# YuanchenBei/ColdRec

Hardware: AMD Instinct MI355X
Metric: ranked items/sec (full-catalogue eval) (higher is better)
Workload: dtype f32; 1 GPU; configs[3] full-catalogue eval: 1000000-row user table x 10000000 items, d=128, k=20, f32 tables, user block 131072 per step, rated CSR (mean ~50) + 20% cold-item bitmap ('warm' setting), item table row-sharded over 1 GPU(s); items=10000000, dim=128, k=20, parallelism=single GPU

## Files before the change

### coldrec_amd/csrc/score_topk.hip

```cpp
#include <math.h>
#include <stdarg.h>
#include <stdlib.h>

#include <algorithm>
#include <atomic>
#include <vector>

#include "score_topk_common.h"

using namespace crh_score;

namespace {

__device__ __forceinline__ bool pack_row_masked(const uint32_t* bitmap, int64_t gid) {
    return bitmap != nullptr && ((bitmap[gid >> 5] >> (gid & 31)) & 1u);
}

template <int D>
__global__ __launch_bounds__(256) void pack_items_kernel(const float* __restrict__ v, int64_t n_items,
                                                         float* __restrict__ packed, const uint32_t* __restrict__ bitmap,
                                                         int64_t item_base) {
    constexpr int NCH = D / 8;
    __shared__ float tile[32][D + 4];
    const int64_t t = blockIdx.x;
// ... 949 lines not shown
        unsigned long long t0 = ~0ull, t1 = 0;
        for (int64_t wv = 0; wv < n_waves; ++wv) { t0 = std::min(t0, h[2 * wv]); t1 = std::max(t1, h[2 * wv + 1]); }
        std::vector<double> st_(n_waves), en_(n_waves);
        for (int64_t wv = 0; wv < n_waves; ++wv) { st_[wv] = (double)(h[2 * wv] - t0); en_[wv] = (double)(h[2 * wv + 1] - t0); }
        std::sort(st_.begin(), st_.end());
        std::sort(en_.begin(), en_.end());
        const double tot = (double)(t1 - t0);
        fprintf(stderr, "[crh timing] waves=%lld span=%.0f ticks; start quantiles 0/25/50/75/100%%: %.3f %.3f %.3f %.3f %.3f; "
                        "end quantiles 0/10/25/50/75/90/100%%: %.3f %.3f %.3f %.3f %.3f %.3f %.3f (fraction of span)\n",
                (long long)n_waves, tot, st_[0] / tot, st_[n_waves / 4] / tot, st_[n_waves / 2] / tot,
                st_[3 * n_waves / 4] / tot, st_[n_waves - 1] / tot, en_[0] / tot, en_[n_waves / 10] / tot,
                en_[n_waves / 4] / tot, en_[n_waves / 2] / tot, en_[3 * n_waves / 4] / tot, en_[9 * n_waves / 10] / tot,
                en_[n_waves - 1] / tot);
        std::vector<double> in_(n_waves), lp_(n_waves), so_(n_waves);
        double ev_ticks = 0, ev = 0, lp_sum = 0;
        for (int64_t wv = 0; wv < n_waves; ++wv) {
            in_[wv] = (double)(h[2 * n_waves + 2 * wv] - h[2 * wv]);
            lp_[wv] = (double)(h[2 * n_waves + 2 * wv + 1] - h[2 * n_waves + 2 * wv]);
            so_[wv] = (double)(h[2 * wv + 1] - h[2 * n_waves + 2 * wv + 1]);
            ev_ticks += (double)h[4 * n_waves + 2 * wv];
            ev += (double)h[4 * n_waves + 2 * wv + 1];
            lp_sum += lp_[wv];
        }
        std::sort(in_.begin(), in_.end());
        std::sort(lp_.begin(), lp_.end());
        std::sort(so_.begin(), so_.end());
        fprintf(stderr, "[crh timing] median ticks: list setup %.0f, tile loop %.0f, list store %.0f; %.0f slow-path events per wave, "
                        "%.0f ticks each = %.3f of the loop\n",
                in_[n_waves / 2], lp_[n_waves / 2], so_[n_waves / 2], ev / (double)n_waves, ev > 0 ? ev_ticks / ev : 0.0,
                lp_sum > 0 ? ev_ticks / lp_sum : 0.0);
    return CRH_OK;
}
int dma_timing_begin(ScoreArgs& a, hipStream_t st) {
    CRH_HIP(hipMalloc(&a.wave_clock, (size_t)16 * 4 * 68 * 8));
    CRH_HIP(hipMemsetAsync(a.wave_clock, 0, (size_t)16 * 4 * 68 * 8, st));
    return CRH_OK;
}
int dma_timing_report(ScoreArgs& a, int esz, int d, hipStream_t st) {
    CRH_HIP(hipStreamSynchronize(st));
    std::vector<unsigned long long> h((size_t)16 * 4 * 68);
    CRH_HIP(hipMemcpy(h.data(), a.wave_clock, h.size() * 8, hipMemcpyDeviceToHost));
    CRH_HIP(hipFree(a.wave_clock));
    {
        unsigned long long tk = 0, ne = 0;
        for (int q = 0; q < 64; ++q) { tk += h[(size_t)16 * 4 * 64 + 2 * q]; ne += h[(size_t)16 * 4 * 64 + 2 * q + 1]; }
        fprintf(stderr, "[crh dma timing] events: %.0f per wave, %.0f cycles each (tiles with at least one candidate; 64 waves)\n",
                (double)ne / 64.0, ne ? (double)tk / (double)ne : 0.0);
    }
    unsigned long long trip_tk = 0, trip_n = 0, loop_cycles = 0;
    for (int wv = 0; wv < 4; ++wv) {
        unsigned long long tot = 0, wsum = 0;
        std::vector<unsigned long long> b(64, 0);
        for (int blk = 0; blk < 16; ++blk)
            for (int q = 0; q < 64; ++q) b[q] += h[((size_t)blk * 4 + wv) * 64 + q];
        const unsigned long long bw = (esz == 4 ? 512 : 128) >> (d * esz == 256 ? 1 : 0);
        for (int q = 0; q < 64; ++q) { tot += b[q]; wsum += b[q] * (q * bw + bw / 2); }
        fprintf(stderr, "[crh dma timing] wave %d: %llu tiles, mean %.0f cycles; histogram (%llu-cycle buckets from 0):", wv, tot,
                tot ? (double)wsum / (double)tot : 0.0, bw);
        for (int q = 0; q < 64; ++q) fprintf(stderr, " %llu", b[q]);
        fprintf(stderr, "\n");
        loop_cycles += 2 * wsum;
    }
    for (int q = 0; q < 64; ++q) { trip_tk += h[(size_t)16 * 4 * 66 + 2 * q]; trip_n += h[(size_t)16 * 4 * 66 + 2 * q + 1]; }
    fprintf(stderr, "[crh dma timing] memory trips inside events (filter hit -> list bounds + search): %.0f per wave, %.0f cycles each, "
                    "%.0f cycles per wave = %.4f of the timed tile loop (64 waves)\n",
            (double)trip_n / 64.0, trip_n ? (double)trip_tk / (double)trip_n : 0.0, (double)trip_tk / 64.0,
            loop_cycles ? (double)trip_tk / (double)loop_cycles : 0.0);
    a.wave_clock = nullptr;
    return CRH_OK;
}
#endif

int score_topk_impl(int esz, const void* user_emb, const int32_t* users, int64_t n_users, const void* item_emb,
                    int64_t n_items, int d, const int64_t* rated_rowptr, const int32_t* rated_col,
                    const uint32_t* cand_bitmap, int k, int64_t item_base, float* out_score, int32_t* out_idx,
                    void* workspace, size_t workspace_bytes, void* stream, int n_splits, void* ev_kernel_start,
                    void* ev_kernel_stop, const char* who, const float* seed_score, const int32_t* seed_idx) {
    CRH_CHECK_ARG(user_emb && item_emb && out_score && out_idx, "%s: NULL table/output pointer", who);
    CRH_CHECK_ARG(n_users > 0 && n_items > 0, "%s: empty block (n_users=%lld, n_items=%lld)", who,
                  (long long)n_users, (long long)n_items);
    CRH_CHECK_ARG(k >= 1 && k <= CRH_MAX_K, "%s: k=%d outside 1..%d", who, k, CRH_MAX_K);
    CRH_CHECK_ARG(esz == 4 ? crh_score_topk_supports_dim(d) : crh_score_topk_f16_supports_dim(d),
                  "%s: d=%d unsupported (pad the tables to %s16/32/64/128/256)", who, d, esz == 4 ? "8/" : "");
    CRH_CHECK_ARG(((uintptr_t)user_emb & 15) == 0 && ((uintptr_t)item_emb & 15) == 0,
                  "%s: tables must be 16-byte aligned", who);
    CRH_CHECK_ARG((rated_rowptr == nullptr) == (rated_col == nullptr) || rated_rowptr != nullptr,
                  "%s: rated_col given without rated_rowptr", who);
    CRH_CHECK_ARG(item_base >= 0 && item_base + n_items < (int64_t)CRH_PAD_IDX, "%s: item ids exceed int32", who);
    CRH_CHECK_ARG(n_splits >= 0 && n_splits <= 64, "%s: n_splits=%d outside 0..64", who, n_splits);

    const RoutePlan rp = plan_route(esz, n_users, n_items, d, k, workspace != nullptr, workspace_bytes, cand_bitmap != nullptr,
                                    n_splits, seed_score != nullptr);
    ScoreArgs a = {};
    a.user_emb = user_emb;
    a.users = users;
    a.n_users = n_users;
    a.item_emb = item_emb;
    a.n_items = n_items;
    a.rated_rowptr = rated_rowptr;
    a.rated_col = rated_col;
// ... 280 lines not shown
        a.out_idx = reinterpret_cast<int32_t*>(a.out_score + (size_t)a.n_splits * n_users * KP);
    }
    static const int sync_win_raw = CRH_TUNE_ENV("CRH_SCORE_SYNC_WINDOW") ? atoi(CRH_TUNE_ENV("CRH_SCORE_SYNC_WINDOW")) : 128;
    static const int sync_win = sync_win_raw <= 0 ? 0 : std::max(2, sync_win_raw & ~1);
    if (sync_win > 0 && a.n_splits == 1 && n_wg <= 256 && n_wg > 8) {
        const int64_t n_win = (T + 1 + sync_win - 1) / sync_win + 1;
        if ((size_t)(n_win + 1) * 8 * sizeof(unsigned) <= sync_bytes(n_items)) {
            a.sync_window = sync_win;
            a.sync_stride = n_win + 1;
            a.xcd_sync = reinterpret_cast<unsigned*>(ws + L.sync);
            CRH_HIP(hipMemsetAsync(a.xcd_sync, 0, (size_t)a.sync_stride * 8 * sizeof(unsigned), st));
        }
    }
    if (compact) {
        a.idmap = stream_map;
        a.n_live = s.stats + SCREEN_STAT_LIVE;
        if (plan.rated_tiles) {
            int32_t* inv = reinterpret_cast<int32_t*>(ws + L.inv);
            uint32_t* rt = reinterpret_cast<uint32_t*>(ws + L.rtiles);
            rc = launch_screen_invmap(stream_map, a.n_live, item_base + P, n_main, inv, st);
            if (rc != CRH_OK) return rc;
            rc = launch_screen_rated_tiles(rated_rowptr, rated_col, n_users, cand_bitmap, item_base + P, item_base + n_items, inv, rt, st);
            if (rc != CRH_OK) return rc;
            a.rated_tiles = rt;
        }
    } else if (cand_bitmap) {
        a.tile_bits = tbits;
    }
#ifdef CRH_PROFILE
    static const int timing = CRH_PROFILE_ENV("CRH_SCORE_TIMING");
    if (timing) {
        rc = dma_timing_begin(a, st);
        if (rc != CRH_OK) return rc;
    }
#endif
    rc = launch_score_dma(2, D, 3, a, st);
    if (rc != CRH_OK) return rc;
#ifdef CRH_PROFILE
    if (timing) {
        rc = dma_timing_report(a, 2, D, st);
        if (rc != CRH_OK) return rc;
    }
#endif
    if (a.n_splits > 1) {
        rc = crh_merge_topk(a.out_score, a.out_idx, a.n_splits, n_users, KP, KP, cand_s, cand_i, stream);
        if (rc != CRH_OK) return rc;
    }

    rc = launch_screen_certify(s, st);
    if (rc != CRH_OK) return rc;
    if (ev_kernel_stop) CRH_HIP(hipEventRecord(reinterpret_cast<hipEvent_t>(ev_kernel_stop), st));
    return CRH_OK;
}
}

namespace {
size_t full_workspace_bytes(int64_t n_users, int64_t n_items, int d, int k, int esz, bool dim_ok) {
    if (n_users <= 0 || k <= 0) return 0;
    const size_t lists = lists_bytes(n_users, k);
    const size_t fused = dim_ok && n_items > 0 ? fused_layout(n_users, n_items, d, k, esz).need : lists;
    size_t need = std::max(fused, dense_block_bytes(n_users, n_items) + (fused - lists));
    const int64_t P = dim_ok ? seed_route(esz, n_users, n_items, d) : 0;
    if (P > 0) need = std::max(need, dense_block_bytes(n_users, P) + packed_bytes(P, d, esz)) + seed_bytes(n_users, k);
    return need;
}
}
// ... 224 lines not shown
```

### coldrec_amd/csrc/score_topk_dma.hip

```cpp
#include <type_traits>
#include <utility>

#include "score_topk_common.h"

namespace crh_score {
namespace {

constexpr int DMA_NW = 4;
constexpr int DMA_UPW = 128;
constexpr int TBITS_B = 2 * 64 * 4;
constexpr int FLAGS_B = 64;
constexpr int IDS_SLOTS = 8;
constexpr int IDS_B = (IDS_SLOTS + 1) * 32 * 4;
constexpr int RT_B = 2 * 256;

constexpr int DMA_FW = 6;
__host__ __device__ constexpr size_t dma_wave_lds_bytes(int K) {
    return (size_t)DMA_UPW * K * 8 + (size_t)DMA_UPW * 4 + (size_t)DMA_UPW * DMA_FW * 4;
}
__device__ __forceinline__ unsigned rated_hash192(int gi) { return ((((unsigned)gi * 2654435761u) >> 16) * (32u * DMA_FW)) >> 16; }

template <int K>
__device__ __forceinline__ float f4_comp(const f32x4& v) {
    if constexpr (K == 0) return v.x;
// ... 99 lines not shown
            lsu[p] = sc;
            liu[p] = gi;
            cnt[ul] = n2;
        }
        if (n2 >= K) {
            const float prev = __builtin_bit_cast(float, __builtin_amdgcn_readlane(__builtin_bit_cast(int, es), K >= 2 ? K - 2 : 0));
            const float kth = (p == K - 1) ? sc : prev;
            const float t = dma_new_tau<MG>(kth, es, sc, a.screen_k < 2 ? 2 : a.screen_k, margin);
            if (mine) tau_reg = t;
        }
    }
}

#ifdef CRH_DMA_EVENT_REBALLOT
constexpr bool DMA_EVENT_REBALLOT = true;
#else
constexpr bool DMA_EVENT_REBALLOT = false;
#endif
#ifdef CRH_DMA_SCREEN_TWO_TRIP
constexpr bool DMA_SCREEN_ONE_TRIP = false;
#else
constexpr bool DMA_SCREEN_ONE_TRIP = true;
#endif
#ifdef CRH_DMA_SCREEN_MFMA32
constexpr bool DMA_SCREEN_M16 = false;
#else
constexpr bool DMA_SCREEN_M16 = true;
#endif
#ifdef CRH_DMA_M16_BODY_OLD
constexpr bool DMA_M16_HOOKED = false;
#else
constexpr bool DMA_M16_HOOKED = true;
#endif
#ifdef CRH_DMA_EVENT_RUNTIME_K
constexpr int DMA_EVENT_KC = 0;
#else
constexpr int DMA_EVENT_KC = SCREEN_KP;
#endif
#ifdef CRH_DMA_EVENT_SLOT_TEST
constexpr bool DMA_EVENT_SLOT_TEST = true;
#else
constexpr bool DMA_EVENT_SLOT_TEST = false;
#endif
#ifdef CRH_DMA_EVENT_TAIL64
constexpr bool DMA_EVENT_TAIL64 = true;
#else
constexpr bool DMA_EVENT_TAIL64 = false;
#endif
#ifdef CRH_DMA_EVENT_MASK8_SPLIT
[[maybe_unused]] constexpr bool DMA_EVENT_MASK8_SPLIT = true;
#else
[[maybe_unused]] constexpr bool DMA_EVENT_MASK8_SPLIT = false;
#endif
#ifdef CRH_DMA_EVENT_NO_FULL
constexpr bool DMA_EVENT_FULL = false;
#else
constexpr bool DMA_EVENT_FULL = DMA_EVENT_KC != 0 && DMA_SCREEN_ONE_TRIP;
#endif
#ifdef CRH_DMA_EVENT_NO_STRAIGHT
constexpr bool DMA_EVENT_STRAIGHT = false;
#else
constexpr bool DMA_EVENT_STRAIGHT = true;
#endif
template <int K, bool RT>
__device__ __forceinline__ void dma_candidate_full(float sc, int gi, bool bm_masked, int ul, int64_t slot, float* ls, int* li,
                                                   const ScoreArgs& a, int lane, const unsigned* rfilter, bool mine, float& tau_reg,
// ... 160 lines not shown
    while (lanes) {
        const int L = __builtin_ctzll(lanes);
        lanes &= lanes - 1;
        unsigned cmL = __builtin_amdgcn_readlane(cm, L);
        const unsigned bmL = __builtin_amdgcn_readlane(bm, L);
        if constexpr (DMA_EVENT_SLOT_TEST) {
            if (slot0 + (L & 15) >= a.n_users) continue;
        }
        while (cmL) {
            const int r = __builtin_ctz(cmL);
            cmL &= cmL - 1;
            candidate(L, r, bmL);
        }
    }
}


template <typename T, int D, int R, bool FL, bool CM = false, bool M16 = false>
__global__ __launch_bounds__(256, 1) void score_topk_dma_kernel(ScoreArgs a) {
    constexpr int NW = DMA_NW, UW = 4, UPW = DMA_UPW;
    static_assert(!M16 || (std::is_same<T, _Float16>::value && D == 128 && !FL), "the 16x16x32 form is the fp16 d=128 screen's");
    constexpr int UB = M16 ? 16 : 32, NU = UPW / UB, NR = M16 ? 8 : 16;
    using AccT = std::conditional_t<M16, f32x8, f32x16>;
    constexpr int PF = FL ? 2 : 3;
    static_assert(R == 4 && (!FL || sizeof(T) == 4) && !(CM && FL), "ring shape");
    constexpr int SIDE_B = CM ? IDS_B + RT_B : TBITS_B;
    constexpr int ROWB = D * (int)sizeof(T);
    constexpr int NCH = ROWB / 32;
    constexpr int TILE_B = NCH * 1024;
    constexpr int CPW = NCH / NW;
    constexpr int GR = 2, NG = NCH / GR;
    constexpr int BG = NG / 2 - 1;
    constexpr int TG = M16 ? 2 : 1;
    static_assert(NCH % NW == 0 && NG % 4 == 0 && BG + 2 < NG, "row width not supported by the DMA kernel");
    extern __shared__ __attribute__((aligned(16))) char smem[];

    const int lane = threadIdx.x & 63;
    const int wave = __builtin_amdgcn_readfirstlane((int)(threadIdx.x >> 6));
    const int S = a.n_splits;
    const int split = (int)(blockIdx.x % S);
    const int64_t ug_raw = (int64_t)(blockIdx.x / S) * NW + wave;
    const bool live = ug_raw < a.n_ugroups;
    const int64_t ug = live ? ug_raw : a.n_ugroups - 1;
    constexpr int KC = M16 ? DMA_EVENT_KC : 0;
    const int K = KC ? KC : a.k;
    const int i = lane & (M16 ? 15 : 31), h = lane >> (M16 ? 4 : 5);
    constexpr bool MG = std::is_same<T, _Float16>::value && D == 128;

    char* ring = smem;
    unsigned* tbits = reinterpret_cast<unsigned*>(smem + R * TILE_B);
    [[maybe_unused]] unsigned* rtiles = tbits + IDS_B / 4;
    unsigned* flags = tbits + SIDE_B / 4;
    if constexpr (FL) {
        if (threadIdx.x < 16) flags[threadIdx.x] = threadIdx.x < PF - 1 ? (unsigned)NW : 0u;
    }
    int64_t n_rows = a.n_items;
    if constexpr (CM) n_rows = (int64_t)__builtin_amdgcn_readfirstlane((int)*a.n_live);
    const int64_t NT = (n_rows + 31) >> 5;
    const int64_t t0 = NT * split / S, t1 = NT * (split + 1) / S;
    const int64_t split_end = (t1 << 5) < n_rows ? (t1 << 5) : n_rows;
    const int64_t slot0w = ug * UPW;
    auto cut_ids = [&](int& lo, int& hi) __attribute__((always_inline)) {
        if constexpr (CM) {
            const int id_end = (int)(a.item_base + a.n_items);
            if (S == 1) {
                lo = (int)a.item_base;
// ... 195 lines not shown
    auto flag_bump = [&](int word) __attribute__((always_inline)) {
#if defined(__HIP_DEVICE_COMPILE__)
        asm volatile("ds_add_u32 %0, %1" ::"v"(flags_lds + 4u * (unsigned)word), "v"(bump_val) : "memory");
#endif
    };
    auto flag_land = [&](unsigned& f) __attribute__((always_inline)) {
#if defined(__HIP_DEVICE_COMPILE__)
        asm volatile("s_waitcnt lgkmcnt(0)" : "+v"(f));
#endif
    };
    auto lds_wait_fl = [&](f32x4(&x)[GR], unsigned& f0, unsigned& f1) __attribute__((always_inline)) {
#if defined(__HIP_DEVICE_COMPILE__)
        asm volatile("s_waitcnt lgkmcnt(%4)" : "+v"(x[0]), "+v"(x[1]), "+v"(f0), "+v"(f1) : "i"(GR));
#endif
    };
    auto flag_spin = [&](unsigned have, int word, unsigned want) __attribute__((always_inline)) {
        unsigned v = __builtin_amdgcn_readfirstlane(have);
        if (__builtin_expect(v >= want, 1) || (CRH_ABLATE(a.ablate) & 4)) return;
        unsigned spins = 0;
        do {
            __builtin_amdgcn_s_sleep(1);
            unsigned t;
#if defined(__HIP_DEVICE_COMPILE__)
            asm volatile("ds_read_b32 %0, %1\n\ts_waitcnt lgkmcnt(0)" : "=v"(t) : "v"(flags_lds + 4u * (unsigned)word) : "memory");
#endif
            v = __builtin_amdgcn_readfirstlane(t);
            if (++spins > (1u << 24)) __builtin_trap();
        } while (v < want);
    };

#ifdef CRH_PROFILE
    unsigned long long ev_ticks = 0, ev_count = 0;
    DmaTripProf tp = {0ull, 0ull};
#endif
    auto event16 = [&](const AccT& v, float& tau_u, int u, int64_t ts, int rows_left, int gi0, unsigned tb, int idv, bool rt) __attribute__((always_inline)) {
        if constexpr (M16) {
            if constexpr (FULL_FORM) {
                if (lists_full) {
                    tile_slow_path_dma16<CM, KC, true>(v, tau_u, ls, li, cnt, K, UB * u, slot0w + UB * u, a, ts << 5, split_end, rows_left, gi0,
                                                       lane, tb, rfilter, idv, margin, rt CRH_TRIP_ARG);
                    return;
                }
            }
            tile_slow_path_dma16<CM, KC>(v, tau_u, ls, li, cnt, K, UB * u, slot0w + UB * u, a, ts << 5, split_end, rows_left, gi0, lane, tb,
                                         rfilter, idv, margin, rt CRH_TRIP_ARG);
        }
    };
    auto body = [&](auto Pc, int j, int s_cur, int s_nxt, int s_fill) __attribute__((always_inline)) {
        constexpr int P = decltype(Pc)::value, Q = 1 - P;
        const uint32_t src = ring_lds + s_cur * TILE_B, srcn = ring_lds + s_nxt * TILE_B;
        float m[NU];
        auto group = [&](auto Gc) __attribute__((always_inline)) {
            constexpr int g = decltype(Gc)::value;
            if constexpr (g + 2 < NG) lds_group(c[(g + 2) & 3], src, std::integral_constant<int, g + 2>{});
            else lds_group(c[(g + 2) & 3], srcn, std::integral_constant<int, g + 2 - NG>{});
            if constexpr (!FL && g == BG) {
                dma_wait_but_newest_tile();
                if (!(CRH_ABLATE(a.ablate) & 4)) __builtin_amdgcn_s_barrier();
            }
            __builtin_amdgcn_sched_barrier(0);
            if constexpr (FL) {
                lds_wait_fl(c[g & 3], rflag, dflag);
            } else {
                lds_wait(c[g & 3], std::integral_constant<int, 2 * GR>{});
            }
            if constexpr (!FL && g == BG) {
// ... 117 lines not shown
                    if constexpr (CM) idv = (int)tbits[((j - 1) & (IDS_SLOTS - 1)) * 32 + (lane & 31)];
                    bool rt = false;
                    if constexpr (CM) rt = (__builtin_amdgcn_readfirstlane(rtiles[(int)((ts >> 9) & 1) * 64 + (int)((ts >> 3) & 63)]) >> (4 * (int)(ts & 7) + wave)) & 1u;
                    const int64_t rl64 = split_end - (ts << 5);
                    const int rows_left = rl64 < 32 ? (int)rl64 : 32;
                    const int gi0 = (int)(a.item_base + (ts << 5));
#pragma unroll
                    for (int u = 0; u < NU; ++u)
                        if ((M16 && !DMA_EVENT_REBALLOT) ? hitb[u] != 0ull : __ballot(m[u] > tau[u]) != 0ull) {
                            if constexpr (M16)
                                event16(acc[Q][u], tau[u], u, ts, rows_left, gi0, tb, idv, rt);
                            else
                                tile_slow_path_dma<sizeof(T) == 4 && DMA_ONE_TRIP_F32, CM, MG>(acc[Q][u], tau[u], ls, li, cnt, K, 32 * u, slot0w + 32 * u, a,
                                                                                                ts << 5, split_end, lane, tb, rfilter, idv, margin, rt CRH_TRIP_ARG);
                        }
                    __builtin_amdgcn_s_waitcnt(0xc07f);
#ifdef CRH_PROFILE
                    if (a.wave_clock != nullptr) {
                        ev_ticks += __builtin_amdgcn_s_memtime() - ev_t0;
                        ev_count += 1;
                    }
#endif
                }
            }
        };
        [&]<int... Gs>(std::integer_sequence<int, Gs...>) __attribute__((always_inline)) {
            (group(std::integral_constant<int, Gs>{}), ...);
        }(std::make_integer_sequence<int, NG>{});
    };

    uint32_t ring_a = ring_lds;
    int next_sync = 0;
    bool sync_due = false;
    auto lds_read1 = [&](f32x4& dst, uint32_t addr, auto Oc) __attribute__((always_inline)) {
#if defined(__HIP_DEVICE_COMPILE__)
        asm volatile("ds_read_b128 %0, %1 offset:%2" : "=v"(dst) : "v"(addr), "i"(decltype(Oc)::value));
#endif
    };
    auto body16 = [&](auto Pc, auto Fc, int j) __attribute__((always_inline)) {
        constexpr int P = decltype(Pc)::value, Q = 1 - P;
        constexpr bool FIRST = decltype(Fc)::value;
        constexpr int LA = P ? 0 : TILE_B;
        static_assert(CPW == 2 || !M16, "two pieces per wave");
        float m[NU], a0[NU], a1[NU], a2[NU];
        unsigned long long hitm = 0ull;
        unsigned long long hitb[NU];
        int tc = 0, tf = 0;
        const unsigned* side = nullptr;
        const char* gt = nullptr;
        auto hook = [&](auto Gc, auto Nc) __attribute__((always_inline)) {
            constexpr int g = decltype(Gc)::value, n = decltype(Nc)::value;
            if constexpr (g == 0 && !FIRST) {
#if defined(__HIP_DEVICE_COMPILE__)
                constexpr int u = n >> 1;
                const AccT& v = acc[Q][u];
                if constexpr ((n & 1) == 0) {
                    asm volatile("v_max3_f32 %0, %1, %2, %3" : "=v"(a0[u]) : "v"(v[0]), "v"(v[1]), "v"(v[2]));
                    asm volatile("v_max3_f32 %0, %1, %2, %3" : "=v"(a1[u]) : "v"(v[3]), "v"(v[4]), "v"(v[5]));
                } else {
                    asm volatile("v_max3_f32 %0, %1, %2, %3" : "=v"(a2[u]) : "v"(v[6]), "v"(v[7]), "v"(a0[u]));
                    asm volatile("v_max_f32 %0, %1, %2" : "=v"(m[u]) : "v"(a1[u]), "v"(a2[u]));
                }
#endif
            }
            if constexpr (g == BG) {
                if constexpr (n == 0) {
                    tc = (int)t0 + j + 3;
                    tc = tc < n_tiles32 ? tc : n_tiles32 - 1;
                    tf = (CRH_ABLATE(a.ablate) & 2) ? 0 : tc;
                }
                if constexpr (n == 1) {
                    if constexpr (CM) {
                        unsigned e = ((unsigned)tc << 5) + (unsigned)lane;
                        const unsigned e_max = ((unsigned)n_tiles32 << 5) - 1u;
                        e = e < e_max ? e : e_max;
                        side = reinterpret_cast<const unsigned*>(a.idmap) + e;
                    } else {
                        int t = ((int)((t0 + j + 32) >> 6) << 6) + lane;
                        t = t < n_tiles32 ? t : n_tiles32 - 1;
                        side = reinterpret_cast<const unsigned*>(a.tile_bits) + (unsigned)t;
                    }
                }
                if constexpr (n == 2) {
                    unsigned* dst = CM ? tbits + ((j + 3) & (IDS_SLOTS - 1)) * 32 : tbits + (((t0 + j + 32) >> 6) & 1) * 64;
                    __builtin_amdgcn_global_load_lds((const __attribute__((address_space(1))) void*)side,
                                                     (__attribute__((address_space(3))) void*)dst, 4, 0, 0);
                }
                if constexpr (n == 3) gt = my_pieces + (int64_t)tf * TILE_B;
                if constexpr (n == 4 || n == 5) {
                    char* l = ring + ((j + 3) & (R - 1)) * TILE_B + (wave * CPW) * 1024;
                    __builtin_amdgcn_global_load_lds((const __attribute__((address_space(1))) void*)gt,
                                                     (__attribute__((address_space(3))) void*)l, 16, (n - 4) * 1024, 0);
                }
                if constexpr (n == 8) lds_read1(c[3][0], ring_a, std::integral_constant<int, P * TILE_B + 3 * 2048>{});
                if constexpr (n == 9) lds_read1(c[3][1], ring_a, std::integral_constant<int, P * TILE_B + 3 * 2048 + 256>{});
                if constexpr (n == 10 && P == 1) ring_a = ring_lds + (unsigned)((j + 1) & 2) * TILE_B;
            }
            if constexpr (g == TG) {
                if constexpr (n < NU && !FIRST) {
                    hitb[n] = __ballot(m[n] > tau[n]);
                    hitm |= hitb[n];
                }
                if constexpr (n == 8) lds_read1(c[0][0], ring_a, std::integral_constant<int, LA>{});
                if constexpr (n == 9) lds_read1(c[0][1], ring_a, std::integral_constant<int, LA + 256>{});
            }
            if constexpr (g == 3) {
                if constexpr (n == 0) lds_read1(c[1][0], ring_a, std::integral_constant<int, LA + 2048>{});
                if constexpr (n == 1) lds_read1(c[1][1], ring_a, std::integral_constant<int, LA + 2048 + 256>{});
                if constexpr (n == 6) lds_read1(c[2][0], ring_a, std::integral_constant<int, LA + 2 * 2048>{});
                if constexpr (n == 7) lds_read1(c[2][1], ring_a, std::integral_constant<int, LA + 2 * 2048 + 256>{});
                if constexpr (n == 8 && P == 1) sync_due = (j + 1 >= next_sync) & (j + 1 < n_steps);
            }
        };
        auto group = [&](auto Gc) __attribute__((always_inline)) {
            constexpr int g = decltype(Gc)::value;
            if constexpr (g == BG) {
                dma_wait_but_newest_tile();
                if (!(CRH_ABLATE(a.ablate) & 4)) __builtin_amdgcn_s_barrier();
            }
            __builtin_amdgcn_sched_barrier(0);
            if constexpr (g == 0) lds_wait(c[g], std::integral_constant<int, 4>{});
            else lds_wait(c[g], std::integral_constant<int, 2>{});
            __builtin_amdgcn_sched_barrier(0);
            [&]<int... N>(std::integer_sequence<int, N...>) __attribute__((always_inline)) {
                (([&]() __attribute__((always_inline)) {
                     constexpr int mb = N >> 3, u = N & 7;
                     AccT& x = acc[P][u];
                     f32x4 t = mb ? f32x4{x[4], x[5], x[6], x[7]} : f32x4{x[0], x[1], x[2], x[3]};
                     if constexpr (g == 0) t = f32x4{0.0f, 0.0f, 0.0f, 0.0f};
                     t = __builtin_amdgcn_mfma_f32_16x16x32_f16(__builtin_bit_cast(f16x8, c[g][mb]), __builtin_bit_cast(f16x8, b[g][u]), t, 0, 0, 0);
#pragma unroll
                     for (int r = 0; r < 4; ++r) x[4 * mb + r] = t[r];
                     __builtin_amdgcn_sched_barrier(0);
                     hook(Gc, std::integral_constant<int, N>{});
                     __builtin_amdgcn_sched_barrier(0);
                 }()),
                 ...);
            }(std::make_integer_sequence<int, 16>{});
            if constexpr (g == TG && !FIRST) {
                if (hitm != 0ull && !(CRH_ABLATE(a.ablate) & 1)) {
#ifdef CRH_PROFILE
                    const unsigned long long ev_t0 = a.wave_clock != nullptr ? __builtin_amdgcn_s_memtime() : 0ull;
#endif
                    const int64_t ts = t0 + j - 1;
                    const unsigned tb = has_bits ? tbits[((ts >> 6) & 1) * 64 + (ts & 63)] : 0u;
                    int idv = 0;
                    if constexpr (CM) idv = (int)tbits[((j - 1) & (IDS_SLOTS - 1)) * 32 + (lane & 31)];
                    bool rt = false;
                    if constexpr (CM) rt = (__builtin_amdgcn_readfirstlane(rtiles[(int)((ts >> 9) & 1) * 64 + (int)((ts >> 3) & 63)]) >> (4 * (int)(ts & 7) + wave)) & 1u;
                    const int64_t rl64 = split_end - (ts << 5);
                    const int rows_left = rl64 < 32 ? (int)rl64 : 32;
                    const int gi0 = (int)(a.item_base + (ts << 5));
#pragma unroll
                    for (int u = 0; u < NU; ++u)
                        if (!DMA_EVENT_REBALLOT ? hitb[u] != 0ull : __ballot(m[u] > tau[u]) != 0ull)
                            if constexpr (M16)
                                event16(acc[Q][u], tau[u], u, ts, rows_left, gi0, tb, idv, rt);
                    __builtin_amdgcn_s_waitcnt(0xc07f);
#ifdef CRH_PROFILE
                    if (a.wave_clock != nullptr) {
                        ev_ticks += __builtin_amdgcn_s_memtime() - ev_t0;
                        ev_count += 1;
                    }
#endif
                }
            }
        };
        [&]<int... Gs>(std::integer_sequence<int, Gs...>) __attribute__((always_inline)) {
            (group(std::integral_constant<int, Gs>{}), ...);
        }(std::make_integer_sequence<int, NG>{});
    };

    if (n_steps > 0) {
        if constexpr (CM) {
            dma_ids(0);
// ... 15 lines not shown
        lds_group(c[0], ring_lds, std::integral_constant<int, 0>{});
        lds_group(c[1], ring_lds, std::integral_constant<int, 1>{});
        if constexpr (FL) flag_read(dflag, 8 + (PF & (R - 1)));
        int s0 = 0;
        unsigned* sync_cnt = nullptr;
        int win_steps = 0;
        next_sync = n_steps + 4;
        if (a.xcd_sync && wave == 0) {
            const unsigned xcc = __builtin_amdgcn_s_getreg(20 | (0 << 6) | (3 << 11)) & 7u;
            sync_cnt = a.xcd_sync + (int64_t)xcc * a.sync_stride;
            if (lane == 0) __hip_atomic_fetch_add(sync_cnt, 1u, __ATOMIC_RELAXED, __HIP_MEMORY_SCOPE_AGENT);
            win_steps = a.sync_window & ~1;
            if (win_steps < 2) win_steps = 2;
            next_sync = 0;
        }
        [[maybe_unused]] int next_win = next_sync, next_rt = n_steps + 4;
        if constexpr (CM) {
            if (rt_fetch && wave == 0) next_rt = (int)(((((t0 >> 9) + 1) << 9) + 64) - t0);
            next_sync = next_win < next_rt ? next_win : next_rt;
        }
#ifdef CRH_PROFILE
        unsigned long long t_prev = 0;
#endif
        auto trip_head = [&](int j, bool due) __attribute__((always_inline)) {
#ifdef CRH_PROFILE
            if (a.wave_clock != nullptr && blockIdx.x < 16) {
                const unsigned long long t_now = __builtin_amdgcn_s_memtime();
                if (j >= 64 && lane == 0) {
                    unsigned long long dt = (t_now - t_prev) >> ((sizeof(T) == 4 ? 10 : 8) - (ROWB == 256 ? 1 : 0));
                    if (dt > 63) dt = 63;
                    atomicAdd(&a.wave_clock[((size_t)blockIdx.x * 4 + wave) * 64 + dt], 1ull);
                }
                t_prev = t_now;
            }
#endif
            auto window = [&](int& nxt) __attribute__((always_inline)) {
                const int win = j / win_steps;
                if (xcd_window_sync(sync_cnt, win, lane)) {
                    nxt += win_steps;
                } else {
                    nxt = n_steps + 4;
                    const int n_win = (n_steps + win_steps - 1) / win_steps;
                    if (lane == 0)
                        for (int wdw = win; wdw < n_win; ++wdw)
                            __hip_atomic_fetch_add(sync_cnt + 1 + wdw, 1u, __ATOMIC_RELAXED, __HIP_MEMORY_SCOPE_AGENT);
                }
            };
            if (due) {
                if constexpr (CM) {
                    if (j >= next_rt) {
                        dma_rtiles(((t0 + j) >> 9) + 1);
                        next_rt += 512;
                    }
                    if (j >= next_win) window(next_win);
                    next_sync = next_win < next_rt ? next_win : next_rt;
                } else {
                    window(next_sync);
                }
            }
        };
        if constexpr (M16 && DMA_M16_HOOKED) {
            lds_group(c[2], ring_lds, std::integral_constant<int, 2>{});
            trip_head(0, 0 >= next_sync);
            body16(std::integral_constant<int, 0>{}, std::true_type{}, 0);
            for (int j = 1;; j += 2) {
                body16(std::integral_constant<int, 1>{}, std::false_type{}, j);
                if (j + 1 > n_steps) break;
                trip_head(j + 1, sync_due);
                body16(std::integral_constant<int, 0>{}, std::false_type{}, j + 1);
                if (j + 2 > n_steps) break;
            }
        } else {
            for (int j = 0; j <= n_steps; j += 2) {
                trip_head(j, j >= next_sync && j < n_steps);
                const int s1 = (s0 + 1) & (R - 1), s2 = (s0 + 2) & (R - 1);
                body(std::integral_constant<int, 0>{}, j, s0, s1, (s0 + PF) & (R - 1));
                if (j + 1 > n_steps) break;
                body(std::integral_constant<int, 1>{}, j + 1, s1, s2, (s1 + PF) & (R - 1));
                s0 = s2;
            }
        }
        dma_wait_all();
#if defined(__HIP_DEVICE_COMPILE__)
        asm volatile("s_waitcnt lgkmcnt(0)" : "+v"(c[0][0]), "+v"(c[0][1]), "+v"(c[1][0]), "+v"(c[1][1]), "+v"(c[2][0]), "+v"(c[2][1]),
                     "+v"(c[3][0]), "+v"(c[3][1]), "+v"(rflag), "+v"(dflag));
#endif
    }

#ifdef CRH_PROFILE
    if (a.wave_clock != nullptr && blockIdx.x < 16 && lane == 0) {
        a.wave_clock[(size_t)16 * 4 * 64 + ((size_t)blockIdx.x * 4 + wave) * 2] = ev_ticks;
        a.wave_clock[(size_t)16 * 4 * 64 + ((size_t)blockIdx.x * 4 + wave) * 2 + 1] = ev_count;
        a.wave_clock[(size_t)16 * 4 * 66 + ((size_t)blockIdx.x * 4 + wave) * 2] = tp.ticks;
        a.wave_clock[(size_t)16 * 4 * 66 + ((size_t)blockIdx.x * 4 + wave) * 2 + 1] = tp.count;
    }
#endif
    if (live) {
        int id_lo, id_hi;
        cut_ids(id_lo, id_hi);
        for (int j = 0; j < UPW; ++j) {
            const int64_t slot = slot0w + j;
            if (slot >= a.n_users) break;
            const int n = __builtin_amdgcn_readfirstlane(cnt[j]);
            const int64_t o = ((int64_t)split * a.n_users + slot) * K;
            if (a.seed_score && S > 1)
                wave_list_store_range(ls + j * K, li + j * K, n, K, a.out_score + o, a.out_idx + o, lane,
                                      split == 0 ? INT32_MIN : id_lo, id_hi);
            else
                wave_list_store(ls + j * K, li + j * K, n, K, a.out_score + o, a.out_idx + o, lane);
        }
    }
}

template <typename T, int D, int R, bool FL, bool CM = false, bool M16 = false>
int launch_score_dma_t(const ScoreArgs& a, hipStream_t stream) {
    const size_t lds = score_dma_lds_bytes(D * (int)sizeof(T), a.k, R, FL, CM);
    auto kern = score_topk_dma_kernel<T, D, R, FL, CM, M16>;
    CRH_HIP(hipFuncSetAttribute(reinterpret_cast<const void*>(kern), hipFuncAttributeMaxDynamicSharedMemorySize,
                                (int)lds));
    const int64_t blocks = ((a.n_ugroups + DMA_NW - 1) / DMA_NW) * a.n_splits;
    hipLaunchKernelGGL(kern, dim3((unsigned)blocks), dim3(64 * DMA_NW), lds, stream, a);
    CRH_HIP(hipGetLastError());
    return CRH_OK;
}

}

// ... 23 lines not shown
```

Before: 6765 billion items/s.

## Carry prefetch addresses across DMA tile loop and straighten rare-path branches

The M16 hooked DMA scoring loop now carries the next tile, side-id and ring addresses in registers and advances them incrementally, instead of recomputing clamped tile indices each step. The trip/sync check is folded into one scalar flag computed in the body, so the loop has a single predicted-rare branch. The event test is marked unlikely, one max3 reduction is fused into a single asm block, and the LDS wait no longer pins accumulator registers. Profiling segment stamps are added behind compile and environment flags. The aim is to cut scalar overhead and branch cost per tile pair, at the cost of tricky address bookkeeping at the end of the range.

```diff
diff --git a/coldrec_amd/csrc/score_topk.hip b/coldrec_amd/csrc/score_topk.hip
--- a/coldrec_amd/csrc/score_topk.hip
+++ b/coldrec_amd/csrc/score_topk.hip
@@ -1005,13 +1005,13 @@
     return CRH_OK;
 }
 int dma_timing_begin(ScoreArgs& a, hipStream_t st) {
-    CRH_HIP(hipMalloc(&a.wave_clock, (size_t)16 * 4 * 68 * 8));
-    CRH_HIP(hipMemsetAsync(a.wave_clock, 0, (size_t)16 * 4 * 68 * 8, st));
+    CRH_HIP(hipMalloc(&a.wave_clock, (size_t)16 * 4 * 80 * 8));
+    CRH_HIP(hipMemsetAsync(a.wave_clock, 0, (size_t)16 * 4 * 80 * 8, st));
     return CRH_OK;
 }
 int dma_timing_report(ScoreArgs& a, int esz, int d, hipStream_t st) {
     CRH_HIP(hipStreamSynchronize(st));
-    std::vector<unsigned long long> h((size_t)16 * 4 * 68);
+    std::vector<unsigned long long> h((size_t)16 * 4 * 80);
     CRH_HIP(hipMemcpy(h.data(), a.wave_clock, h.size() * 8, hipMemcpyDeviceToHost));
     CRH_HIP(hipFree(a.wave_clock));
     {
@@ -1039,6 +1039,22 @@
                     "%.0f cycles per wave = %.4f of the timed tile loop (64 waves)\n",
             (double)trip_n / 64.0, trip_n ? (double)trip_tk / (double)trip_n : 0.0, (double)trip_tk / 64.0,
             loop_cycles ? (double)trip_tk / (double)loop_cycles : 0.0);
+    {
+        unsigned long long pairs = 0, seg[10] = {0, 0, 0, 0, 0, 0, 0, 0, 0, 0};
+        for (int q = 0; q < 64; ++q) {
+            pairs += h[(size_t)16 * 4 * 68 + (size_t)q * 11];
+            for (int sg = 0; sg < 10; ++sg) seg[sg] += h[(size_t)16 * 4 * 68 + (size_t)q * 11 + 1 + sg];
+        }
+        if (pairs) {
+            static const char* const nm[5] = {"group 0", "dma wait + barrier", "group 1", "group 2 + event test", "group 3 + trip edge"};
+            double sum = 0;
+            for (int sg = 0; sg < 10; ++sg) sum += (double)seg[sg] / (double)pairs;
+            fprintf(stderr, "[crh dma timing] segments of a pair without an event (%.0f pairs per wave, mean cycles; stamped, so longer than the "
+                            "histogram's tiles): pair %.0f =", (double)pairs / 64.0, sum);
+            for (int sg = 0; sg < 10; ++sg)
+                fprintf(stderr, " %s %s %.1f%s", sg < 5 ? "even" : "odd", nm[sg % 5], (double)seg[sg] / (double)pairs, sg == 9 ? "\n" : ",");
+        }
+    }
     a.wave_clock = nullptr;
     return CRH_OK;
 }
@@ -1385,6 +1401,7 @@
     if (timing) {
         rc = dma_timing_begin(a, st);
         if (rc != CRH_OK) return rc;
+        if (timing >= 2) a.ablate |= 32;
     }
 #endif
     rc = launch_score_dma(2, D, 3, a, st);
diff --git a/coldrec_amd/csrc/score_topk_dma.hip b/coldrec_amd/csrc/score_topk_dma.hip
--- a/coldrec_amd/csrc/score_topk_dma.hip
+++ b/coldrec_amd/csrc/score_topk_dma.hip
@@ -155,6 +155,22 @@
 #else
 constexpr bool DMA_M16_HOOKED = true;
 #endif
+#ifdef CRH_DMA_BODY_PADDED
+constexpr bool DMA_BODY_PADDED = true;
+#else
+constexpr bool DMA_BODY_PADDED = false;
+#endif
+#ifdef CRH_DMA_BODY_RECOMPUTE
+constexpr bool DMA_BODY_CARRY = false;
+#else
+constexpr bool DMA_BODY_CARRY = true;
+#endif
+#ifdef CRH_DMA_BODY_BRANCHY
+constexpr bool DMA_BODY_STRAIGHT = false;
+#else
+constexpr bool DMA_BODY_STRAIGHT = true;
+#endif
+#define CRH_DMA_BODY_RARE(straight, x) ((straight) ? __builtin_expect(!!(x), 0) : (long)!!(x))
 #ifdef CRH_DMA_EVENT_RUNTIME_K
 constexpr int DMA_EVENT_KC = 0;
 #else
@@ -381,6 +397,7 @@
     constexpr int GR = 2, NG = NCH / GR;
     constexpr int BG = NG / 2 - 1;
     constexpr int TG = M16 ? 2 : 1;
+    constexpr bool BODY_CARRY = DMA_BODY_CARRY && CM, BODY_STRAIGHT = DMA_BODY_STRAIGHT && CM;
     static_assert(NCH % NW == 0 && NG % 4 == 0 && BG + 2 < NG, "row width not supported by the DMA kernel");
     extern __shared__ __attribute__((aligned(16))) char smem[];
 
@@ -642,6 +659,21 @@
 #ifdef CRH_PROFILE
     unsigned long long ev_ticks = 0, ev_count = 0;
     DmaTripProf tp = {0ull, 0ull};
+    unsigned seg_tmp[10] = {0, 0, 0, 0, 0, 0, 0, 0, 0, 0}, seg_sum[10] = {0, 0, 0, 0, 0, 0, 0, 0, 0, 0}, seg_pairs = 0;
+    unsigned long long seg_prev = 0;
+    bool seg_ev = false;
+#ifdef CRH_DMA_BODY_STAMPS
+    const bool seg_on = a.wave_clock != nullptr && blockIdx.x < 16 && (a.ablate & 32);
+#else
+    constexpr bool seg_on = false;
+#endif
+    auto seg_stamp = [&](auto Kc) __attribute__((always_inline)) {
+        if (seg_on) {
+            const unsigned long long t = __builtin_amdgcn_s_memtime();
+            seg_tmp[decltype(Kc)::value] = (unsigned)(t - seg_prev);
+            seg_prev = t;
+        }
+    };
 #endif
     auto event16 = [&](const AccT& v, float& tau_u, int u, int64_t ts, int rows_left, int gi0, unsigned tb, int idv, bool rt) __attribute__((always_inline)) {
         if constexpr (M16) {
@@ -825,6 +857,26 @@
     uint32_t ring_a = ring_lds;
     int next_sync = 0;
     bool sync_due = false;
+    [[maybe_unused]] const char* f_tile = nullptr;
+    [[maybe_unused]] const char* f_side = nullptr;
+    [[maybe_unused]] unsigned f_soff = 0, f_sx = 0, f_ids = 0, f_ring = 0;
+    [[maybe_unused]] int f_jl = 0;
+    [[maybe_unused]] unsigned tb_lds = (unsigned)(uintptr_t)(__attribute__((address_space(3))) unsigned*)tbits;
+    [[maybe_unused]] unsigned lane4 = (unsigned)lane * 4u, lane16 = (unsigned)lane * 16u;
+    [[maybe_unused]] int trip_rare = 0;
+#if defined(__HIP_DEVICE_COMPILE__)
+    if constexpr (M16 && DMA_M16_HOOKED && BODY_CARRY) {
+        asm volatile("" : "+v"(lane4));
+        asm volatile("" : "+v"(lane16));
+        asm volatile("" : "+s"(tb_lds));
+    }
+#endif
+    auto lds_wait_bare = [&](auto Nc) __attribute__((always_inline)) {
+#if defined(__HIP_DEVICE_COMPILE__)
+        if (CRH_ABLATE(a.ablate) & 8) return;
+        asm volatile("s_waitcnt lgkmcnt(%0)" ::"i"(decltype(Nc)::value));
+#endif
+    };
     auto lds_read1 = [&](f32x4& dst, uint32_t addr, auto Oc) __attribute__((always_inline)) {
 #if defined(__HIP_DEVICE_COMPILE__)
         asm volatile("ds_read_b128 %0, %1 offset:%2" : "=v"(dst) : "v"(addr), "i"(decltype(Oc)::value));
@@ -838,9 +890,11 @@
         float m[NU], a0[NU], a1[NU], a2[NU];
         unsigned long long hitm = 0ull;
         unsigned long long hitb[NU];
-        int tc = 0, tf = 0;
-        const unsigned* side = nullptr;
-        const char* gt = nullptr;
+        [[maybe_unused]] int tc = 0, tf = 0;
+        [[maybe_unused]] const unsigned* side = nullptr;
+        [[maybe_unused]] const char* gt = nullptr;
+        [[maybe_unused]] unsigned inc = 0, inct = 0;
+        [[maybe_unused]] auto umin = [](unsigned x, unsigned y) __attribute__((always_inline)) { return x < y ? x : y; };
         auto hook = [&](auto Gc, auto Nc) __attribute__((always_inline)) {
             constexpr int g = decltype(Gc)::value, n = decltype(Nc)::value;
             if constexpr (g == 0 && !FIRST) {
@@ -850,13 +904,67 @@
                 if constexpr ((n & 1) == 0) {
                     asm volatile("v_max3_f32 %0, %1, %2, %3" : "=v"(a0[u]) : "v"(v[0]), "v"(v[1]), "v"(v[2]));
                     asm volatile("v_max3_f32 %0, %1, %2, %3" : "=v"(a1[u]) : "v"(v[3]), "v"(v[4]), "v"(v[5]));
-                } else {
+                } else if constexpr (DMA_BODY_PADDED) {
                     asm volatile("v_max3_f32 %0, %1, %2, %3" : "=v"(a2[u]) : "v"(v[6]), "v"(v[7]), "v"(a0[u]));
                     asm volatile("v_max_f32 %0, %1, %2" : "=v"(m[u]) : "v"(a1[u]), "v"(a2[u]));
-                }
-#endif
-            }
-            if constexpr (g == BG) {
+                } else {
+                    asm volatile("v_max3_f32 %0, %1, %2, %3\n\tv_max_f32 %0, %4, %0"
+                                 : "=&v"(m[u])
+                                 : "v"(v[6]), "v"(v[7]), "v"(a0[u]), "v"(a1[u]));
+                }
+#endif
+            }
+            if constexpr (g == BG && BODY_CARRY) {
+#if defined(__HIP_DEVICE_COMPILE__)
+                if constexpr (n == 0)
+                    __builtin_amdgcn_global_load_lds((const __attribute__((address_space(1))) void*)(f_side + f_soff),
+                                                     (__attribute__((address_space(3))) void*)(uintptr_t)(tb_lds + f_ids), 4, 0, 0);
+                if constexpr (n == 1 || n == 2) {
+                    asm volatile("" : "+v"(lane16));
+                    __builtin_amdgcn_global_load_lds((const __attribute__((address_space(1))) void*)(f_tile + lane16),
+                                                     (__attribute__((address_space(3))) void*)(ring + f_ring + (wave * CPW) * 1024), 16,
+                                                     (n - 1) * 1024, 0);
+                }
+                if constexpr (n == 2) {
+                    f_soff = umin(lane4, f_sx);
+                    asm volatile("" : "+v"(f_soff));
+                }
+                if constexpr (n == 3) {
+                    inc = j < f_jl ? 128u : 0u;
+                    asm volatile("" : "+s"(inc));
+                }
+                if constexpr (n == 4) {
+                    f_side += inc;
+                    asm volatile("" : "+s"(f_side));
+                }
+                if constexpr (n == 5) {
+                    f_sx = j < f_jl - 2 ? 252u : 124u;
+                    asm volatile("" : "+s"(f_sx));
+                }
+                if constexpr (n == 6) {
+                    inct = inc << 6;
+                    static_assert(TILE_B == 64 * 128 || !M16, "the tile's step is 64 times the ids'");
+                    if (CRH_ABLATE(a.ablate) & 2) inct = 0u;
+                    asm volatile("" : "+s"(inct));
+                }
+                if constexpr (n == 7) {
+                    f_tile += inct;
+                    asm volatile("" : "+s"(f_tile));
+                }
+                if constexpr (n == 8) lds_read1(c[3][0], ring_a, std::integral_constant<int, P * TILE_B + 3 * 2048>{});
+                if constexpr (n == 9) lds_read1(c[3][1], ring_a, std::integral_constant<int, P * TILE_B + 3 * 2048 + 256>{});
+                if constexpr (n == 10 && P == 1) ring_a = ring_lds + (f_ring ^ (unsigned)(2 * TILE_B));
+                if constexpr (n == 11) {
+                    f_ids = (f_ids + 128u) & (unsigned)(IDS_SLOTS * 128 - 1);
+                    asm volatile("" : "+s"(f_ids));
+                }
+                if constexpr (n == 12) {
+                    f_ring = (f_ring + (unsigned)TILE_B) & (unsigned)(R * TILE_B - 1);
+                    asm volatile("" : "+s"(f_ring));
+                }
+#endif
+            }
+            if constexpr (g == BG && !BODY_CARRY) {
                 if constexpr (n == 0) {
                     tc = (int)t0 + j + 3;
                     tc = tc < n_tiles32 ? tc : n_tiles32 - 1;
@@ -903,17 +1011,40 @@
                 if constexpr (n == 6) lds_read1(c[2][0], ring_a, std::integral_constant<int, LA + 2 * 2048>{});
                 if constexpr (n == 7) lds_read1(c[2][1], ring_a, std::integral_constant<int, LA + 2 * 2048 + 256>{});
                 if constexpr (n == 8 && P == 1) sync_due = (j + 1 >= next_sync) & (j + 1 < n_steps);
+                if constexpr (n == 9 && BODY_STRAIGHT && !FIRST) {
+#if defined(__HIP_DEVICE_COMPILE__)
+                    int rare;
+                    if constexpr (P == 1)
+                        asm volatile("s_min_i32 %0, %1, %2\n\ts_cmp_ge_i32 %3, %0\n\ts_cselect_b32 %0, 1, 0"
+                                     : "=&s"(rare) : "s"(next_sync), "s"(n_steps + 1), "s"(j + 1) : "scc");
+                    else
+                        asm volatile("s_cmp_gt_i32 %1, %2\n\ts_cselect_b32 %0, 1, 0" : "=s"(rare) : "s"(j + 1), "s"(n_steps) : "scc");
+                    trip_rare = rare;
+#endif
+                }
             }
         };
         auto group = [&](auto Gc) __attribute__((always_inline)) {
             constexpr int g = decltype(Gc)::value;
+#ifdef CRH_PROFILE
+            if constexpr (g == 0) seg_stamp(std::integral_constant<int, 5 * (1 - P) + 4>{});
+            else if constexpr (g == BG) seg_stamp(std::integral_constant<int, 5 * P + 0>{});
+            else seg_stamp(std::integral_constant<int, 5 * P + g>{});
+#endif
             if constexpr (g == BG) {
                 dma_wait_but_newest_tile();
                 if (!(CRH_ABLATE(a.ablate) & 4)) __builtin_amdgcn_s_barrier();
+#ifdef CRH_PROFILE
+                seg_stamp(std::integral_constant<int, 5 * P + 1>{});
+#endif
             }
             __builtin_amdgcn_sched_barrier(0);
-            if constexpr (g == 0) lds_wait(c[g], std::integral_constant<int, 4>{});
-            else lds_wait(c[g], std::integral_constant<int, 2>{});
+            if constexpr (DMA_BODY_PADDED) {
+                if constexpr (g == 0) lds_wait(c[g], std::integral_constant<int, 4>{});
+                else lds_wait(c[g], std::integral_constant<int, 2>{});
+            } else {
+                lds_wait_bare(std::integral_constant<int, g == 0 ? 4 : 2>{});
+            }
             __builtin_amdgcn_sched_barrier(0);
             [&]<int... N>(std::integer_sequence<int, N...>) __attribute__((always_inline)) {
                 (([&]() __attribute__((always_inline)) {
@@ -931,9 +1062,10 @@
                  ...);
             }(std::make_integer_sequence<int, 16>{});
             if constexpr (g == TG && !FIRST) {
-                if (hitm != 0ull && !(CRH_ABLATE(a.ablate) & 1)) {
+                if (CRH_DMA_BODY_RARE(BODY_STRAIGHT, hitm != 0ull && !(CRH_ABLATE(a.ablate) & 1))) {
 #ifdef CRH_PROFILE
                     const unsigned long long ev_t0 = a.wave_clock != nullptr ? __builtin_amdgcn_s_memtime() : 0ull;
+                    seg_ev = true;
 #endif
                     const int64_t ts = t0 + j - 1;
                     const unsigned tb = has_bits ? tbits[((ts >> 6) & 1) * 64 + (ts & 63)] : 0u;
@@ -1015,6 +1147,12 @@
                     atomicAdd(&a.wave_clock[((size_t)blockIdx.x * 4 + wave) * 64 + dt], 1ull);
                 }
                 t_prev = t_now;
+                if (seg_on && j >= 64 && !seg_ev) {
+#pragma unroll
+                    for (int q = 0; q < 10; ++q) seg_sum[q] += seg_tmp[q];
+                    seg_pairs += 1;
+                }
+                seg_ev = false;
             }
 #endif
             auto window = [&](int& nxt) __attribute__((always_inline)) {
@@ -1044,14 +1182,38 @@
         };
         if constexpr (M16 && DMA_M16_HOOKED) {
             lds_group(c[2], ring_lds, std::integral_constant<int, 2>{});
+            if constexpr (BODY_CARRY) {
+                const int last = n_tiles32 - 1, t3 = (int)t0 + 3;
+                const int tc0 = t3 < last ? t3 : last;
+                f_jl = last - t3;
+                f_tile = packed + (wave * CPW) * 1024 + (int64_t)((CRH_ABLATE(a.ablate) & 2) ? 0 : tc0) * TILE_B;
+                f_ring = 3u * (unsigned)TILE_B;
+                f_side = reinterpret_cast<const char*>(a.idmap) + (int64_t)tc0 * 128;
+                const unsigned lim0 = t3 < last ? 252u : 124u;
+                f_soff = lane4 < lim0 ? lane4 : lim0;
+                f_sx = t3 + 1 < last ? 252u : 124u;
+                f_ids = 3u * 128u;
+            }
             trip_head(0, 0 >= next_sync);
             body16(std::integral_constant<int, 0>{}, std::true_type{}, 0);
             for (int j = 1;; j += 2) {
                 body16(std::integral_constant<int, 1>{}, std::false_type{}, j);
-                if (j + 1 > n_steps) break;
-                trip_head(j + 1, sync_due);
-                body16(std::integral_constant<int, 0>{}, std::false_type{}, j + 1);
-                if (j + 2 > n_steps) break;
+                if constexpr (BODY_STRAIGHT) {
+                    if (CRH_DMA_BODY_RARE(BODY_STRAIGHT, trip_rare != 0)) {
+                        if (j + 1 > n_steps) break;
+                        trip_head(j + 1, sync_due);
+                    }
+#ifdef CRH_PROFILE
+                    else trip_head(j + 1, false);
+#endif
+                    body16(std::integral_constant<int, 0>{}, std::false_type{}, j + 1);
+                    if (CRH_DMA_BODY_RARE(BODY_STRAIGHT, trip_rare != 0)) break;
+                } else {
+                    if (j + 1 > n_steps) break;
+                    trip_head(j + 1, sync_due);
+                    body16(std::integral_constant<int, 0>{}, std::false_type{}, j + 1);
+                    if (j + 2 > n_steps) break;
+                }
             }
         } else {
             for (int j = 0; j <= n_steps; j += 2) {
@@ -1076,6 +1238,8 @@
         a.wave_clock[(size_t)16 * 4 * 64 + ((size_t)blockIdx.x * 4 + wave) * 2 + 1] = ev_count;
         a.wave_clock[(size_t)16 * 4 * 66 + ((size_t)blockIdx.x * 4 + wave) * 2] = tp.ticks;
         a.wave_clock[(size_t)16 * 4 * 66 + ((size_t)blockIdx.x * 4 + wave) * 2 + 1] = tp.count;
+        a.wave_clock[(size_t)16 * 4 * 68 + ((size_t)blockIdx.x * 4 + wave) * 11] = seg_pairs;
+        for (int q = 0; q < 10; ++q) a.wave_clock[(size_t)16 * 4 * 68 + ((size_t)blockIdx.x * 4 + wave) * 11 + 1 + q] = seg_sum[q];
     }
 #endif
     if (live) {
```

New measurement: 6968 billion items/s, median of 6. 1.03x the previous value.
